# dremovd/PPO

Measured on AMD Instinct MI355X. Metric: env-steps/sec (Pong-shaped synthetic, 256 envs/GPU), higher is better.
Workload: dtype f32

## Files before the change

### ppo_amd/csrc/stack_fused.hip

```cpp
#include <cstdlib>
#include <type_traits>

#include "common.h"
#include "conv_stage.h"
#include "mfma.h"

#ifndef PPO_TAIL_SPLIT
#define PPO_TAIL_SPLIT 2
#endif

namespace ppo {
namespace {

constexpr int kScrPitchS = 20;

struct StackTailArgs {
    const float *in;
    const float *w[4];
    const float *bias[4];
    const float *mask[4];
    float *save[4];
    int n_images;
};

template <int C, int H, int W, int MT, int NW, int NSPLIT>
struct StackCfg {
    static constexpr int ROWS = H + 2;
    static constexpr int G = 4;
    static constexpr int PLANE_RAW = ROWS * W + 2 * G;
    static constexpr int PLANE = PLANE_RAW + ((16 - PLANE_RAW % 32) + 32) % 32;
    static constexpr int NT = C / 16;
    static constexpr int NTL = NT / NSPLIT;
    static constexpr int WAVES = NW * NSPLIT;
    static constexpr int KS = 9 * (C / 4);
    static constexpr int NPIX = H * W;
    static constexpr int MTILES = (NPIX + 15) / 16;
    static constexpr int LDS_MAP = C * PLANE;
    static constexpr size_t LDS_BYTES = (size_t)2 * LDS_MAP * 4;
    static_assert(C % 16 == 0, "channel tiles of 16");
    static_assert(MTILES == MT * NW, "one group of MT pixel tiles per wave");
    static_assert(NT % NSPLIT == 0, "channel tiles split evenly");
};

template <int C, int H, int W, int MT, int NW, int NSPLIT, bool BACKWARD>
__global__ __launch_bounds__(NW * NSPLIT * 64) void stack_tail_kernel(StackTailArgs a)
{
    using S = StackCfg<C, H, W, MT, NW, NSPLIT>;
    constexpr int NT = S::NTL, KS = S::KS, PLANE = S::PLANE, G = S::G;
    extern __shared__ __align__(16) float smem[];
    const int tid = threadIdx.x, lane = tid & 63, l15 = lane & 15, g = lane >> 4;
    const int wave = (tid >> 6) % NW;
    const int n0 = ((tid >> 6) / NW) * NT;

    zero_lds<2 * S::LDS_MAP, S::WAVES * 64>(smem, tid);
    __syncthreads();

    int pix[MT], lofs[MT];
    float hi_l[MT], hi_r[MT];
#pragma unroll
    for (int m = 0; m < MT; ++m) {
        const int p = (wave * MT + m) * 16 + l15;
        pix[m] = p;
        const int pc = p < S::NPIX ? p : 0;
        lofs[m] = G + pc - 1 + g * PLANE;
        hi_l[m] = (pc % W == 0) ? 0.f : INFINITY;
        hi_r[m] = (pc % W == W - 1) ? 0.f : INFINITY;
    }

    float wa[NT][KS];
    auto load_weights = [&](int layer) {
        const float4 *pw = reinterpret_cast<const float4 *>(a.w[layer]);
#pragma unroll
        for (int s4 = 0; s4 < KS / 4; ++s4)
#pragma unroll
            for (int n = 0; n < NT; ++n) {
                const float4 v = pw[(s4 * S::NT + n0 + n) * 64 + lane];
                wa[n][4 * s4 + 0] = v.x;
                wa[n][4 * s4 + 1] = v.y;
                wa[n][4 * s4 + 2] = v.z;
                wa[n][4 * s4 + 3] = v.w;
            }
    };
    load_weights(0);

    for (int img = blockIdx.x; img < a.n_images; img += gridDim.x) {
        __syncthreads();
        stage_band_chunk_dma<C, H, W, S::ROWS, PLANE, G, S::WAVES>(a.in, img, 0, smem, tid);
        const size_t img_off = (size_t)img * C * H * W;

#pragma unroll 1
        for (int layer = 0; layer < 4; ++layer) {
            float bias_r[NT][4];
#pragma unroll
            for (int n = 0; n < NT; ++n)
#pragma unroll
                for (int r = 0; r < 4; ++r) bias_r[n][r] = BACKWARD ? 0.f : a.bias[layer][(n0 + n) * 16 + g * 4 + r];
            float gate[BACKWARD ? MT : 1][NT][4];
            if constexpr (BACKWARD) {
                const __amdgpu_buffer_rsrc_t mask = buffer_of(a.mask[layer] + img_off);
#pragma unroll
                for (int m = 0; m < MT; ++m)
#pragma unroll
                    for (int n = 0; n < NT; ++n)
#pragma unroll
                        for (int r = 0; r < 4; ++r)
                            gate[m][n][r] = buffer_f32(mask, pix[m] < S::NPIX ? (((n0 + n) * 16 + g * 4 + r) * (H * W) + pix[m]) * 4
                                                                              : kOutside);
            }

            __syncthreads();
            const int odd = layer & 1;
            const int src = odd ? S::LDS_MAP : 0;
            int base[MT];
#pragma unroll
            for (int m = 0; m < MT; ++m) base[m] = lofs[m] + src;

            f32x4 acc[NT][MT];
#pragma unroll
            for (int n = 0; n < NT; ++n)
#pragma unroll
                for (int m = 0; m < MT; ++m) acc[n][m] = f32x4{0.f, 0.f, 0.f, 0.f};

            constexpr int SB = (MT * NT >= 4) ? 2 : 4;
            constexpr int NB = (KS + SB - 1) / SB;
            float raw[2][SB][MT];
            auto load_block = [&](int j, float (&r)[SB][MT]) {
#pragma unroll
                for (int u = 0; u < SB; ++u) {
                    const int s = j * SB + u;
                    if (s < KS) {
                        const int tap = s / (C / 4), cs = s % (C / 4);
                        const int tap_off = (tap / 3) * W + (tap % 3);
#pragma unroll
                        for (int m = 0; m < MT; ++m) r[u][m] = smem[base[m] + cs * 4 * PLANE + tap_off];
                    }
                }
            };
            load_block(0, raw[0]);
#pragma unroll
            for (int j = 0; j < NB; ++j) {
                float bv[SB][MT];
#pragma unroll
                for (int u = 0; u < SB; ++u) {
                    const int s = j * SB + u;
                    if (s < KS) {
                        const int kx = (s / (C / 4)) % 3;
#pragma unroll
                        for (int m = 0; m < MT; ++m) {
                            float x = raw[j & 1][u][m];
                            if (kx != 1) {
                                const float hi = kx == 0 ? hi_l[m] : hi_r[m];
                                x = __builtin_amdgcn_fmed3f(x, BACKWARD ? -hi : 0.f, hi);
                            } else if (!BACKWARD) {
                                x = relu1(x);
                            }
                            bv[u][m] = x;
                        }
                    }
                }
                __builtin_amdgcn_sched_barrier(0);
                if (j + 1 < NB) load_block(j + 1, raw[(j + 1) & 1]);
#pragma unroll
                for (int u = 0; u < SB; ++u) {
                    const int s = j * SB + u;
                    if (s < KS) {
#pragma unroll
                        for (int m = 0; m < MT; ++m)
#pragma unroll
                            for (int n = 0; n < NT; ++n) acc[n][m] = mfma16(wa[n][s], bv[u][m], acc[n][m]);
                    }
                }
                __builtin_amdgcn_sched_barrier(0);
            }

            __builtin_amdgcn_sched_barrier(0);
            load_weights((layer + 1) & 3);
            float *dst = smem + (odd ? 0 : S::LDS_MAP);
            float *save = a.save[layer];
            __builtin_amdgcn_sched_barrier(0);
            float skip[MT][NT][4];
#pragma unroll
            for (int m = 0; m < MT; ++m)
#pragma unroll
                for (int n = 0; n < NT; ++n)
#pragma unroll
                    for (int r = 0; r < 4; ++r)
                        skip[m][n][r] = odd ? smem[((n0 + n) * 16 + g * 4 + r) * PLANE + G + W + (pix[m] < S::NPIX ? pix[m] : 0)] : 0.f;
#pragma unroll
            for (int m = 0; m < MT; ++m) {
                if (pix[m] < S::NPIX) {
#pragma unroll
                    for (int n = 0; n < NT; ++n)
#pragma unroll
                        for (int r = 0; r < 4; ++r) {
                            const int co = (n0 + n) * 16 + g * 4 + r;
                            const int lo = co * PLANE + G + W + pix[m];
                            float val = acc[n][m][r] + bias_r[n][r];
                            if constexpr (BACKWARD) val = gate[m][n][r] > 0.f ? val : 0.f;
                            if (odd) val = val + skip[m][n][r];
                            dst[lo] = val;
                            if (save) save[img_off + (size_t)co * (H * W) + pix[m]] = val;
                        }
                }
            }
        }
    }
}

template <int C, int H, int W, int MT, int NW, int NSPLIT, bool BACKWARD>
int launch_stack_tail(const StackTailArgs &args, hipStream_t st)
{
    using S = StackCfg<C, H, W, MT, NW, NSPLIT>;
    constexpr auto kern = stack_tail_kernel<C, H, W, MT, NW, NSPLIT, BACKWARD>;
    int nb = 0;
    if (int rc = prepare_kernel<kern>("stack_tail", S::LDS_BYTES, S::WAVES * 64, &nb)) return rc;
    const int wg_per_cu = nb < 1 ? 1 : nb;
    int grid = 256 * wg_per_cu;
    if (grid > args.n_images) grid = args.n_images;
    hipLaunchKernelGGL(kern, dim3(grid), dim3(S::WAVES * 64), S::LDS_BYTES, st, args);
    return check_launch("stack_tail_kernel");
}

template <int C, int H, int W, int TR>
struct ShiftCfg {
    static_assert(C == 16, "one channel tile per wave");
    static constexpr int NW = 16;
    static constexpr int GW = 8;
    static constexpr int G = 4;
    static constexpr int ROWS = H + 6;
    static constexpr int PLANE_RAW = ROWS * W + 2 * G;
    static constexpr int PLANE = PLANE_RAW + ((16 - PLANE_RAW % 32) + 32) % 32;
    static constexpr int KS = 9 * (C / 4);
    static constexpr int NBANDS = (H + TR - 1) / TR;
    static constexpr int NPIX = TR * W;
    static constexpr int MTILES = (NPIX + 15) / 16;
    static constexpr int MT = MTILES / GW;
    static constexpr int LDS_MAP = C * PLANE;
    static constexpr int SCR = MT * 16 * kScrPitchS;
    static constexpr size_t LDS_BYTES = (size_t)(LDS_MAP + GW * SCR) * 4;
    static_assert(H % TR == 0 && MTILES == MT * GW, "whole bands, tiles split evenly over a group's waves");
    static_assert((H * W) % 4 == 0 && NPIX % 4 == 0 && W % 2 == 0, "float4 epilogue on whole quads");
    static_assert(LDS_BYTES <= 160 * 1024, "map + scratch must fit the CU's LDS");
};

template <int C, int H, int W, int TR, bool BACKWARD>
__global__ __launch_bounds__(1024) void stack_shift_kernel(StackTailArgs a)
{
    using S = ShiftCfg<C, H, W, TR>;
    constexpr int KS = S::KS, PLANE = S::PLANE, G = S::G, MT = S::MT, NW = S::NW;
    extern __shared__ __align__(16) float smem[];
    const int tid = threadIdx.x, lane = tid & 63, l15 = lane & 15, g = lane >> 4, wave = tid >> 6;
    const int grp = __builtin_amdgcn_readfirstlane(wave / S::GW), wv = wave % S::GW;
    const int ch = lane >> 2, quad = lane & 3;
    float *scr = smem + S::LDS_MAP + wv * S::SCR;

    int lofs[MT], p4[MT];
    float hi_l[MT], hi_r[MT];
#pragma unroll
    for (int m = 0; m < MT; ++m) {
        const int p = (wv * MT + m) * 16 + l15;
        lofs[m] = G + p - 1 + g * PLANE;
        hi_l[m] = (p % W == 0) ? 0.f : INFINITY;
        hi_r[m] = (p % W == W - 1) ? 0.f : INFINITY;
        p4[m] = (wv * MT + m) * 16 + quad * 4;
    }

    for (int img = blockIdx.x; img < a.n_images; img += gridDim.x) {
        const size_t img_off = (size_t)img * C * H * W;
        __syncthreads();
        for (int i = tid; i < C * 6 * W; i += NW * 64) {
            const int c = i / (6 * W), r = (i / W) % 6, x = i % W;
            smem[c * PLANE + G + (r < 5 ? r : H + 5) * W + x] = 0.f;
        }
        for (int i = tid; i < C * 2 * G; i += NW * 64)
            smem[(i / (2 * G)) * PLANE + ((i % (2 * G)) < G ? (i % G) : G + S::ROWS * W + (i % G))] = 0.f;
        {
            using gptr_t = const __attribute__((address_space(1))) void *;
            using lptr_t = __attribute__((address_space(3))) void *;
            constexpr int N4 = H * W / 4, REQ = (N4 + 63) / 64;
            const int w0 = __builtin_amdgcn_readfirstlane(wave);
            for (int c = w0; c < C; c += NW) {
                const float *g0 = a.in + img_off + (size_t)c * H * W;
                float *l0 = smem + c * PLANE + G + 5 * W;
#pragma unroll
                for (int q = 0; q < REQ; ++q)
                    if (q * 64 + lane < N4)
                        __builtin_amdgcn_global_load_lds((gptr_t)(g0 + (q * 64 + lane) * 4), (lptr_t)(l0 + q * 256), 16, 0, 0);
            }
        }

#pragma unroll 1
        for (int layer = 0; layer < 4; ++layer) {
            float wa[KS];
            const float4 *pw = reinterpret_cast<const float4 *>(a.w[layer]);
#pragma unroll
            for (int s4 = 0; s4 < KS / 4; ++s4) {
                const float4 v = pw[s4 * 64 + lane];
                wa[4 * s4 + 0] = v.x, wa[4 * s4 + 1] = v.y, wa[4 * s4 + 2] = v.z, wa[4 * s4 + 3] = v.w;
            }
            const float bias_c = BACKWARD ? 0.f : a.bias[layer][ch];
            const int odd = layer & 1;
            const float *res = odd ? (layer == 1 ? a.in : a.save[1]) + img_off : nullptr;
            const float *mask = BACKWARD ? a.mask[layer] + img_off : nullptr;
            float *save = a.save[layer] ? a.save[layer] + img_off : nullptr;
            const __amdgpu_buffer_rsrc_t mask_b = buffer_of(mask, mask != nullptr), res_b = buffer_of(res, res != nullptr);
            const int in_row = 5 - layer;

            f32x4 acc[MT];
            float4 gate4[MT], res4[MT];

            __syncthreads();
#pragma unroll 1
            for (int hs = 0; hs <= S::NBANDS; ++hs) {
                if ((hs & 1) == grp) {
                    if (hs < S::NBANDS) {
                        const int y0 = hs * TR;
                        const int chan_off = ch * (H * W) + y0 * W;
#pragma unroll
                        for (int m = 0; m < MT; ++m) {
                            const bool live = p4[m] < S::NPIX;
                            const int off = live ? (chan_off + p4[m]) * 4 : kOutside;
                            if constexpr (BACKWARD) gate4[m] = buffer_f32x4(mask_b, off);
                            res4[m] = buffer_f32x4(res_b, off);
                        }
                        int base[MT];
#pragma unroll
                        for (int m = 0; m < MT; ++m) {
                            base[m] = lofs[m] + (y0 - 1 + in_row) * W;
                            acc[m] = f32x4{0.f, 0.f, 0.f, 0.f};
                        }
                        constexpr int SB = 2;
                        constexpr int NB = (KS + SB - 1) / SB;
                        float raw[2][SB][MT];
                        auto load_block = [&](int j, float (&r)[SB][MT]) {
#pragma unroll
                            for (int u = 0; u < SB; ++u) {
                                const int s = j * SB + u;
                                if (s < KS) {
                                    const int tap = s / (C / 4), cs = s % (C / 4);
                                    const int tap_off = (tap / 3) * W + (tap % 3);
#pragma unroll
                                    for (int m = 0; m < MT; ++m) r[u][m] = smem[base[m] + cs * 4 * PLANE + tap_off];
                                }
                            }
                        };
                        load_block(0, raw[0]);
#pragma unroll
                        for (int j = 0; j < NB; ++j) {
                            float bv[SB][MT];
#pragma unroll
                            for (int u = 0; u < SB; ++u) {
                                const int s = j * SB + u;
                                if (s < KS) {
                                    const int kx = (s / (C / 4)) % 3;
#pragma unroll
                                    for (int m = 0; m < MT; ++m) {
                                        float x = raw[j & 1][u][m];
                                        if (kx != 1) {
                                            const float hi = kx == 0 ? hi_l[m] : hi_r[m];
                                            x = __builtin_amdgcn_fmed3f(x, BACKWARD ? -hi : 0.f, hi);
                                        } else if (!BACKWARD) {
                                            x = relu1(x);
                                        }
                                        bv[u][m] = x;
                                    }
                                }
                            }
                            __builtin_amdgcn_sched_barrier(0);
                            if (j + 1 < NB) load_block(j + 1, raw[(j + 1) & 1]);
#pragma unroll
                            for (int u = 0; u < SB; ++u) {
                                const int s = j * SB + u;
                                if (s < KS) {
#pragma unroll
                                    for (int m = 0; m < MT; ++m) acc[m] = mfma16(wa[s], bv[u][m], acc[m]);
                                }
                            }
                            __builtin_amdgcn_sched_barrier(0);
                        }
                    } else if (layer < 3) {
                        for (int i = tid % (S::GW * 64); i < C * W; i += S::GW * 64)
                            smem[(i / W) * PLANE + G + (H + in_row - 1) * W + i % W] = 0.f;
                    }
                } else if (hs >= 1) {
                    const int y0 = (hs - 1) * TR;
                    const int chan_off = ch * (H * W) + y0 * W;
#pragma unroll
                    for (int m = 0; m < MT; ++m)
#pragma unroll
                        for (int r = 0; r < 4; ++r) scr[(m * 16 + g * 4 + r) * kScrPitchS + l15] = acc[m][r];
                    __builtin_amdgcn_wave_barrier();
                    float *out_row = smem + ch * PLANE + G + (y0 + in_row - 1) * W;
#pragma unroll
                    for (int m = 0; m < MT; ++m) {
                        if (p4[m] >= S::NPIX) continue;
                        const float4 o = *reinterpret_cast<const float4 *>(scr + (m * 16 + ch) * kScrPitchS + quad * 4);
                        const float ov[4] = {o.x, o.y, o.z, o.w};
                        const float gv[4] = {gate4[m].x, gate4[m].y, gate4[m].z, gate4[m].w};
                        const float rv[4] = {res4[m].x, res4[m].y, res4[m].z, res4[m].w};
                        float v[4];
#pragma unroll
                        for (int e = 0; e < 4; ++e) {
                            float val = ov[e] + bias_c;
                            if constexpr (BACKWARD) val = gv[e] > 0.f ? val : 0.f;
                            v[e] = val + rv[e];
                        }
                        if (layer < 3) {
                            *reinterpret_cast<float2 *>(out_row + p4[m]) = make_float2(v[0], v[1]);
                            *reinterpret_cast<float2 *>(out_row + p4[m] + 2) = make_float2(v[2], v[3]);
                        }
                        if (save) *reinterpret_cast<float4 *>(save + chan_off + p4[m]) = make_float4(v[0], v[1], v[2], v[3]);
                    }
                    __builtin_amdgcn_wave_barrier();
                }
                __syncthreads();
            }
        }
    }
}

template <int C, int H, int W, int TR, bool BACKWARD>
int launch_stack_shift(const StackTailArgs &args, hipStream_t st)
{
    using S = ShiftCfg<C, H, W, TR>;
    constexpr auto kern = stack_shift_kernel<C, H, W, TR, BACKWARD>;
    if (int rc = prepare_kernel<kern>("stack_shift", S::LDS_BYTES)) return rc;
    int grid = 256;
    if (grid > args.n_images) grid = args.n_images;
    hipLaunchKernelGGL(kern, dim3(grid), dim3(S::NW * 64), S::LDS_BYTES, st, args);
    return check_launch("stack_shift_kernel");
}

template <int I, int N, class F>
__device__ __forceinline__ void static_for(F &&f)
{
    if constexpr (I < N) {
        f(std::integral_constant<int, I>{});
        static_for<I + 1, N>(f);
    }
}

struct LaneMap {
    template <int MT>
    struct T {
        int pix[MT], lofs[MT];
        float hi_l[MT], hi_r[MT];
    };
};

template <int H, int W, int PLANE, int G, int MT>
__device__ __forceinline__ void lane_map_init(LaneMap::T<MT> &lm, int pixel_wave, int l15, int g)
{
#pragma unroll
    for (int m = 0; m < MT; ++m) {
        const int p = (pixel_wave * MT + m) * 16 + l15;
        lm.pix[m] = p;
        const int pc = p < H * W ? p : 0;
        lm.lofs[m] = G + pc - 1 + g * PLANE;
        lm.hi_l[m] = (pc % W == 0) ? 0.f : INFINITY;
        lm.hi_r[m] = (pc % W == W - 1) ? 0.f : INFINITY;
    }
}

template <int C, int H, int W, int MT, int NTOT, int NT, bool RELU_IN, bool GATED = false>
__device__ __forceinline__ void resident_conv(float *smem, int src_off, int dst_off, bool residual, const float *wpk,
                                              const float *bias, float *save, const LaneMap::T<MT> &lm, int n0, int lane,
                                              const float *mask = nullptr)
{
    constexpr int ROWS = H + 2, G = 4, PLANE_RAW = ROWS * W + 2 * G;
    constexpr int PLANE = PLANE_RAW + ((16 - PLANE_RAW % 32) + 32) % 32;
    constexpr int KS = 9 * (C / 4);
    const int g = lane >> 4;
    float wa[NT][KS];
    const float4 *pw = reinterpret_cast<const float4 *>(wpk);
#pragma unroll
    for (int s4 = 0; s4 < KS / 4; ++s4)
#pragma unroll
        for (int n = 0; n < NT; ++n) {
            const float4 v = pw[(s4 * NTOT + n0 + n) * 64 + lane];
            wa[n][4 * s4 + 0] = v.x;
            wa[n][4 * s4 + 1] = v.y;
            wa[n][4 * s4 + 2] = v.z;
            wa[n][4 * s4 + 3] = v.w;
        }
    float bias_r[NT][4];
#pragma unroll
    for (int n = 0; n < NT; ++n)
#pragma unroll
        for (int r = 0; r < 4; ++r) bias_r[n][r] = (GATED || !bias) ? 0.f : bias[(n0 + n) * 16 + g * 4 + r];
    constexpr int SB = (MT * NT >= 4) ? 2 : 4;
    constexpr int NB = (KS + SB - 1) / SB;
    constexpr int GATE_AT = (GATED && MT * NT * 4 > 16) ? NB / 2 : -1;
    float gate[GATED ? MT : 1][NT][4];
    auto load_gate = [&]() {
        const __amdgpu_buffer_rsrc_t mask_b = buffer_of(mask);
#pragma unroll
        for (int m = 0; m < MT; ++m)
#pragma unroll
            for (int n = 0; n < NT; ++n)
#pragma unroll
                for (int r = 0; r < 4; ++r)
                    gate[m][n][r] = buffer_f32(mask_b, lm.pix[m] < H * W ? (((n0 + n) * 16 + g * 4 + r) * (H * W) + lm.pix[m]) * 4
                                                                         : kOutside);
    };
    if constexpr (GATED && GATE_AT < 0) load_gate();

    __syncthreads();
    int base[MT];
#pragma unroll
    for (int m = 0; m < MT; ++m) base[m] = lm.lofs[m] + src_off;
    f32x4 acc[NT][MT];
#pragma unroll
    for (int n = 0; n < NT; ++n)
#pragma unroll
        for (int m = 0; m < MT; ++m) acc[n][m] = f32x4{0.f, 0.f, 0.f, 0.f};

    float raw[2][SB][MT];
    auto load_block = [&](int j, float (&r)[SB][MT]) {
#pragma unroll
        for (int u = 0; u < SB; ++u) {
            const int s = j * SB + u;
            if (s < KS) {
                const int tap = s / (C / 4), cs = s % (C / 4);
                const int tap_off = (tap / 3) * W + (tap % 3);
#pragma unroll
                for (int m = 0; m < MT; ++m) r[u][m] = smem[base[m] + cs * 4 * PLANE + tap_off];
            }
        }
    };
    load_block(0, raw[0]);
    static_for<0, NB>([&](auto jc) {
        constexpr int j = decltype(jc)::value;
        float bv[SB][MT];
#pragma unroll
        for (int u = 0; u < SB; ++u) {
            const int s = j * SB + u;
            if (s < KS) {
                const int kx = (s / (C / 4)) % 3;
#pragma unroll
                for (int m = 0; m < MT; ++m) {
                    float x = raw[j & 1][u][m];
                    if (kx != 1) {
                        const float hi = kx == 0 ? lm.hi_l[m] : lm.hi_r[m];
                        x = __builtin_amdgcn_fmed3f(x, RELU_IN ? 0.f : -hi, hi);
                    } else if (RELU_IN) {
                        x = relu1(x);
                    }
                    bv[u][m] = x;
                }
            }
        }
        __builtin_amdgcn_sched_barrier(0);
        if constexpr (j + 1 < NB) load_block(j + 1, raw[(j + 1) & 1]);
        if constexpr (j == GATE_AT) load_gate();
#pragma unroll
        for (int u = 0; u < SB; ++u) {
            const int s = j * SB + u;
            if (s < KS) {
#pragma unroll
                for (int m = 0; m < MT; ++m)
#pragma unroll
                    for (int n = 0; n < NT; ++n) acc[n][m] = mfma16(wa[n][s], bv[u][m], acc[n][m]);
            }
        }
        __builtin_amdgcn_sched_barrier(0);
    });
#pragma unroll
    for (int m = 0; m < MT; ++m) {
        if (lm.pix[m] < H * W) {
#pragma unroll
            for (int n = 0; n < NT; ++n)
#pragma unroll
                for (int r = 0; r < 4; ++r) {
                    const int co = (n0 + n) * 16 + g * 4 + r;
                    const int lo = dst_off + co * PLANE + G + W + lm.pix[m];
                    float val = acc[n][m][r] + bias_r[n][r];
                    if constexpr (GATED) val = gate[m][n][r] > 0.f ? val : 0.f;
                    if (residual) val = val + smem[lo];
                    smem[lo] = val;
                    if (save) save[(size_t)co * (H * W) + lm.pix[m]] = val;
                }
        }
    }
}

struct StackFullArgs {
    const float *in;
    const float *w[5];
    const float *bias[5];
    float *pooled;
    uint8_t *argmax;
    float *save[4];
    const float *pre_w[4];
    const float *pre_bias[4];
    float *pre_save[4];
    int has_pre;
    int n_images;
};

template <int C, int HI, int WI, int MTI, int HO, int WO, int MTO, int NW, int NSPLIT>
__global__ __launch_bounds__(NW * NSPLIT * 64) void stack_full_kernel(StackFullArgs a)
{
    using SI = StackCfg<C, HI, WI, MTI, NW, NSPLIT>;
    using SO = StackCfg<C, HO, WO, MTO, NW, NSPLIT>;
    static_assert(HO == (HI + 1) / 2 && WO == (WI + 1) / 2, "3x3 / stride 2 / pad 1 pooling");
    static_assert(2 * SO::LDS_MAP <= SI::LDS_MAP, "the small maps reuse the input map's LDS");
    constexpr int NT = SI::NTL, WAVES = SI::WAVES, THREADS = WAVES * 64;
    constexpr int A_OFF = 0, B_OFF = SI::LDS_MAP, X_OFF = 0, Y_OFF = SO::LDS_MAP;
    extern __shared__ __align__(16) float smem[];
    const int tid = threadIdx.x, lane = tid & 63, l15 = lane & 15, g = lane >> 4;
    const int wave = tid >> 6, pixel_wave = wave % NW, n0 = (wave / NW) * NT;

    LaneMap::T<MTI> lmi;
    LaneMap::T<MTO> lmo;
    lane_map_init<HI, WI, SI::PLANE, SI::G, MTI>(lmi, pixel_wave, l15, g);
    lane_map_init<HO, WO, SO::PLANE, SO::G, MTO>(lmo, pixel_wave, l15, g);

    if (a.has_pre) zero_lds<SI::LDS_MAP, THREADS>(smem + B_OFF, tid);

    for (int img = blockIdx.x; img < a.n_images; img += gridDim.x) {
        __syncthreads();
        zero_lds<SI::LDS_MAP, THREADS>(smem + A_OFF, tid);
        __syncthreads();
        stage_band_chunk_dma<C, HI, WI, SI::ROWS, SI::PLANE, SI::G, WAVES>(a.in, img, 0, smem + A_OFF, tid);
        if (a.has_pre) {
            const size_t big_img = (size_t)img * C * HI * WI;
#pragma unroll 1
            for (int layer = 0; layer < 4; ++layer) {
                const int odd = layer & 1;
                float *save = a.pre_save[layer] ? a.pre_save[layer] + big_img : nullptr;
                resident_conv<C, HI, WI, MTI, SI::NT, NT, true>(smem, odd ? B_OFF : A_OFF, odd ? A_OFF : B_OFF, odd != 0,
                                                                a.pre_w[layer], a.pre_bias[layer], save, lmi, n0, lane);
            }
        }
        resident_conv<C, HI, WI, MTI, SI::NT, NT, false>(smem, A_OFF, B_OFF, false, a.w[0], a.bias[0], nullptr, lmi, n0, lane);
        __syncthreads();
        zero_lds<2 * SO::LDS_MAP, THREADS>(smem + X_OFF, tid);
        __syncthreads();
        {
            constexpr int RPW = 64 / WO;
            const int sub = lane / WO, xo = lane % WO;
            const size_t out_img = (size_t)img * C * HO * WO;
            for (int u0 = wave * RPW; u0 < C * HO; u0 += WAVES * RPW) {
                const int u = u0 + sub;
                const int co = u / HO, yo = u % HO;
                if (sub < RPW && co < C) {
                    const float *src = smem + B_OFF + co * SI::PLANE + SI::G + WI + (2 * yo - 1) * WI + 2 * xo - 1;
                    float best;
                    int best_tap;
                    pool_window_lds<HI % 2 == 0, WI % 2 == 0>(src, WI, yo > 0, 2 * yo + 1 < HI, xo > 0, 2 * xo + 1 < WI, best, best_tap);
                    smem[X_OFF + co * SO::PLANE + SO::G + WO + yo * WO + xo] = best;
                    const size_t oi = out_img + ((size_t)co * HO + yo) * WO + xo;
                    if (a.pooled) a.pooled[oi] = best;
                    if (a.argmax) a.argmax[oi] = (uint8_t)best_tap;
                }
            }
        }
        const size_t out_img = (size_t)img * C * HO * WO;
#pragma unroll 1
        for (int layer = 0; layer < 4; ++layer) {
            const int odd = layer & 1;
            float *save = a.save[layer] ? a.save[layer] + out_img : nullptr;
            resident_conv<C, HO, WO, MTO, SO::NT, NT, true>(smem, odd ? Y_OFF : X_OFF, odd ? X_OFF : Y_OFF, odd != 0,
                                                            a.w[1 + layer], a.bias[1 + layer], save, lmo, n0, lane);
        }
    }
}

struct StackFullBwdArgs {
    const float *g;
    const float *w[5];
    const float *mask[4];
    const uint8_t *argmax;
    float *save[4];
    float *dc;
    float *g_prev;
    const float *post_w[4];
    const float *post_mask[4];
    float *post_save[4];
    int has_post;
    int n_images;
};

template <int C, int HI, int WI, int MTI, int HO, int WO, int MTO, int NW, int NSPLIT>
__global__ __launch_bounds__(NW * NSPLIT * 64) void stack_full_bwd_kernel(StackFullBwdArgs a)
{
    using SI = StackCfg<C, HI, WI, MTI, NW, NSPLIT>;
    using SO = StackCfg<C, HO, WO, MTO, NW, NSPLIT>;
    static_assert(2 * SO::LDS_MAP <= SI::LDS_MAP, "the small maps live inside the first big map's LDS");
    static_assert(C * HO * WO <= SO::LDS_MAP * 4, "the argmax bytes of an image fit the second small map");
    constexpr int NT = SI::NTL, WAVES = SI::WAVES, THREADS = WAVES * 64;
    constexpr int A_OFF = 0, B_OFF = SI::LDS_MAP, X_OFF = 0, Y_OFF = SO::LDS_MAP;
    extern __shared__ __align__(16) float smem[];
    const int tid = threadIdx.x, lane = tid & 63, l15 = lane & 15, g = lane >> 4;
    const int wave = tid >> 6, pixel_wave = wave % NW, n0 = (wave / NW) * NT;

    LaneMap::T<MTI> lmi;
    LaneMap::T<MTO> lmo;
    lane_map_init<HI, WI, SI::PLANE, SI::G, MTI>(lmi, pixel_wave, l15, g);
    lane_map_init<HO, WO, SO::PLANE, SO::G, MTO>(lmo, pixel_wave, l15, g);

    zero_lds<SI::LDS_MAP, THREADS>(smem + B_OFF, tid);

    for (int img = blockIdx.x; img < a.n_images; img += gridDim.x) {
        __syncthreads();
        zero_lds<2 * SO::LDS_MAP, THREADS>(smem + X_OFF, tid);
        __syncthreads();
        stage_band_chunk_dma<C, HO, WO, SO::ROWS, SO::PLANE, SO::G, WAVES>(a.g, img, 0, smem + X_OFF, tid);
        const size_t small_img = (size_t)img * C * HO * WO, big_img = (size_t)img * C * HI * WI;
        constexpr int AM_WORDS = C * HO * WO / 4, AM_PER = (AM_WORDS + THREADS - 1) / THREADS;
        static_assert(C * HO * WO % 4 == 0, "an image's argmax bytes are whole words (the entry points check the base)");
        uint32_t am_r[AM_PER];
#pragma unroll
        for (int k = 0; k < AM_PER; ++k) {
            const int i = tid + k * THREADS;
            am_r[k] = reinterpret_cast<const uint32_t *>(a.argmax + small_img)[i < AM_WORDS ? i : 0];
        }
#pragma unroll 1
        for (int layer = 0; layer < 4; ++layer) {
            const int odd = layer & 1;
            resident_conv<C, HO, WO, MTO, SO::NT, NT, false, true>(smem, odd ? Y_OFF : X_OFF, odd ? X_OFF : Y_OFF, odd != 0,
                                                                   a.w[layer], nullptr, a.save[layer] + small_img, lmo, n0,
                                                                   lane, a.mask[layer] + small_img);
        }
        __syncthreads();
        const uint8_t *am = reinterpret_cast<const uint8_t *>(smem + Y_OFF);
#pragma unroll
        for (int k = 0; k < AM_PER; ++k) {
            const int i = tid + k * THREADS;
            if (i < AM_WORDS) reinterpret_cast<uint32_t *>(smem + Y_OFF)[i] = am_r[k];
        }
        __syncthreads();
        {
            for (int e = tid; e < C * HI * WI; e += THREADS) {
                const int co = e / (HI * WI), r = e % (HI * WI);
                const int iy = r / WI, ix = r % WI;
                const int k = ix >> 1, oy0 = iy >> 1;
                const int ky0 = (iy & 1) ? 2 : 1;
                const bool has_oy1 = (iy & 1) && (oy0 + 1 < HO);
                const bool odd_x = ix & 1;
                const bool has_ox1 = odd_x && (k + 1 < WO);
                const int kx0 = odd_x ? 2 : 1;
                const float *gx = smem + X_OFF + co * SO::PLANE + SO::G + WO;
                const uint8_t *ac = am + co * (HO * WO);
                float sum = 0.f;
                {
                    const int i00 = oy0 * WO + k;
                    if (ac[i00] == ky0 * 3 + kx0) sum += gx[i00];
                    if (has_ox1 && ac[i00 + 1] == ky0 * 3 + 0) sum += gx[i00 + 1];
                }
                if (has_oy1) {
                    const int i10 = (oy0 + 1) * WO + k;
                    if (ac[i10] == kx0) sum += gx[i10];
                    if (has_ox1 && ac[i10 + 1] == 0) sum += gx[i10 + 1];
                }
                smem[B_OFF + co * SI::PLANE + SI::G + WI + r] = sum;
                a.dc[big_img + e] = sum;
            }
        }
        if (a.has_post) {
            __syncthreads();
            zero_lds<SI::LDS_MAP, THREADS>(smem + A_OFF, tid);
        }
        resident_conv<C, HI, WI, MTI, SI::NT, NT, false, false>(smem, B_OFF, A_OFF, false, a.w[4], nullptr,
                                                                a.g_prev + big_img, lmi, n0, lane);
        if (a.has_post) {
#pragma unroll 1
            for (int layer = 0; layer < 4; ++layer) {
                const int odd = layer & 1;
                resident_conv<C, HI, WI, MTI, SI::NT, NT, false, true>(smem, odd ? B_OFF : A_OFF, odd ? A_OFF : B_OFF, odd != 0,
                                                                       a.post_w[layer], nullptr, a.post_save[layer] + big_img,
                                                                       lmi, n0, lane, a.post_mask[layer] + big_img);
            }
        }
    }
}

template <int C, int HI, int WI, int MTI, int HO, int WO, int MTO, int NW, int NSPLIT>
int launch_stack_full_bwd(const StackFullBwdArgs &args, hipStream_t st)
{
    using SI = StackCfg<C, HI, WI, MTI, NW, NSPLIT>;
    constexpr size_t kLds = 2 * (size_t)SI::LDS_MAP * 4;
    constexpr auto kern = stack_full_bwd_kernel<C, HI, WI, MTI, HO, WO, MTO, NW, NSPLIT>;
    if (int rc = prepare_kernel<kern>("stack_full_bwd", kLds)) return rc;
    const int grid = args.n_images < 256 ? args.n_images : 256;
    hipLaunchKernelGGL(kern, dim3(grid), dim3(SI::WAVES * 64), kLds, st, args);
    return check_launch("stack_full_bwd_kernel");
}

template <int C, int HI, int WI, int MTI, int HO, int WO, int MTO, int NW, int NSPLIT>
int launch_stack_full(const StackFullArgs &args, hipStream_t st)
{
    using SI = StackCfg<C, HI, WI, MTI, NW, NSPLIT>;
    constexpr size_t kLds = 2 * (size_t)SI::LDS_MAP * 4;
    constexpr auto kern = stack_full_kernel<C, HI, WI, MTI, HO, WO, MTO, NW, NSPLIT>;
    if (int rc = prepare_kernel<kern>("stack_full", kLds)) return rc;
    const int grid = args.n_images < 256 ? args.n_images : 256;
    hipLaunchKernelGGL(kern, dim3(grid), dim3(SI::WAVES * 64), kLds, st, args);
    return check_launch("stack_full_kernel");
}


struct ChainSplitArgs {
    const float *in;
    const float *pre_w[4];
    const float *pre_bias[4];
    const float *w[5];
    const float *bias[5];
    float *out;
    float *xbuf;
    uint32_t *flags;
    uint32_t *ctl;
    int n_images;
    int skip;
};

constexpr int kSplitWaves = 8;
constexpr uint32_t kSpinLimit = 1u << 21;

template <int C, int HI, int WI, int HO, int WO>
__global__ __launch_bounds__(kSplitWaves * 64) void stack_chain_split_kernel(ChainSplitArgs a)
{
    static_assert(C == 32, "two channel tiles: one per workgroup of a pair");
    using SI = StackCfg<C, HI, WI, 7, 4, 2>;
    using SO = StackCfg<C, HO, WO, 2, 4, 2>;
    constexpr int MTI = 4, MTO = 2, WAVES = kSplitWaves, THREADS = WAVES * 64;
    static_assert(SI::MTILES <= MTI * WAVES && SO::MTILES == MTO * 4 && WAVES == 8, "every pixel tile has a wave");
    static_assert(2 * SO::LDS_MAP <= SI::LDS_MAP, "the small maps reuse the input map's LDS");
    constexpr int A_OFF = 0, B_OFF = SI::LDS_MAP, X_OFF = 0, Y_OFF = SO::LDS_MAP;
    extern __shared__ __align__(16) float smem[];
    const int tid = threadIdx.x, lane = tid & 63, l15 = lane & 15, g = lane >> 4;
    const int wave = tid >> 6;
    const int b = blockIdx.x;
    const int h = (b >> 3) & 1;
    const int pair0 = (b & 7) | ((b >> 4) << 3);
    const int n_pairs = (gridDim.x >> 4) << 3;

    LaneMap::T<MTI> lmi;
    LaneMap::T<MTO> lmo;
    lane_map_init<HI, WI, SI::PLANE, SI::G, MTI>(lmi, wave, l15, g);
    lane_map_init<HO, WO, SO::PLANE, SO::G, MTO>(lmo, wave & 3, l15, g);

    const uint32_t base = __hip_atomic_load(a.ctl, __ATOMIC_RELAXED, __HIP_MEMORY_SCOPE_AGENT) * 8u;
    const uint32_t fault = __hip_atomic_load(a.ctl + 3, __ATOMIC_RELAXED, __HIP_MEMORY_SCOPE_AGENT);
    const uint32_t spin_limit = fault ? 1u << 10 : kSpinLimit;
    bool gave_up = false;
    zero_lds<SI::LDS_MAP, THREADS>(smem + B_OFF, tid);

    for (int img = pair0; img < a.n_images; img += n_pairs) {
        uint32_t *flag_own = a.flags + 2 * img + h, *flag_other = a.flags + 2 * img + (1 - h);
        float *slots = a.xbuf + (size_t)img * 2 * C * HI * WI;
        uint32_t step = 0;
        auto exchange = [&](int dst_off, float *slot, bool fetch) {
            ++step;
            asm volatile("s_waitcnt vmcnt(0)" ::: "memory");
            __syncthreads();
            if (tid == 0) {
                if (!(fault && h == 1))
                    __hip_atomic_store(flag_own, base + step, __ATOMIC_RELAXED, __HIP_MEMORY_SCOPE_AGENT);
                uint32_t it = 0;
                while (!(a.skip & 1) && !gave_up &&
                       __hip_atomic_load(flag_other, __ATOMIC_RELAXED, __HIP_MEMORY_SCOPE_AGENT) < base + step) {
                    if (++it > spin_limit ||
                        ((it & 1023u) == 0 && __hip_atomic_load(a.ctl + 2, __ATOMIC_RELAXED, __HIP_MEMORY_SCOPE_AGENT))) {
                        __hip_atomic_store(a.ctl + 2, 1u, __ATOMIC_RELAXED, __HIP_MEMORY_SCOPE_AGENT);
                        gave_up = true;
                        break;
                    }
                    __builtin_amdgcn_s_sleep(2);
                }
            }
            __syncthreads();
            if (fetch)
                stage_band_chunk_dma<16, HI, WI, SI::ROWS, SI::PLANE, SI::G, WAVES, 16>(slot + (size_t)(1 - h) * 16 * HI * WI, 0, 0,
                                                                                       smem + dst_off + (1 - h) * 16 * SI::PLANE, tid);
        };

        __syncthreads();
        zero_lds<SI::LDS_MAP, THREADS>(smem + A_OFF, tid);
        __syncthreads();
        stage_band_chunk_dma<C, HI, WI, SI::ROWS, SI::PLANE, SI::G, WAVES>(a.in, img, 0, smem + A_OFF, tid);
#pragma unroll 1
        for (int layer = 0; layer < 4; ++layer) {
            const int odd = layer & 1;
            float *slot = slots + (size_t)(layer & 1) * C * HI * WI;
            resident_conv<C, HI, WI, MTI, 2, 1, true>(smem, odd ? B_OFF : A_OFF, odd ? A_OFF : B_OFF, odd != 0, a.pre_w[layer],
                                                      a.pre_bias[layer], slot, lmi, h, lane);
            exchange(odd ? A_OFF : B_OFF, slot, true);
        }
        resident_conv<C, HI, WI, MTI, 2, 1, false>(smem, A_OFF, B_OFF, false, a.w[0], a.bias[0], slots, lmi, h, lane);
        exchange(B_OFF, slots, h == 0);
        if (h != 0 || (a.skip & 2)) continue;
        __syncthreads();
        zero_lds<2 * SO::LDS_MAP, THREADS>(smem + X_OFF, tid);
        __syncthreads();
        {
            constexpr int RPW = 64 / WO;
            const int sub = lane / WO, xo = lane % WO;
            for (int u0 = wave * RPW; u0 < C * HO; u0 += WAVES * RPW) {
                const int u = u0 + sub;
                const int co = u / HO, yo = u % HO;
                if (sub < RPW && co < C) {
                    const float *src = smem + B_OFF + co * SI::PLANE + SI::G + WI + (2 * yo - 1) * WI + 2 * xo - 1;
                    float best;
                    int best_tap;
                    pool_window_lds<HI % 2 == 0, WI % 2 == 0>(src, WI, yo > 0, 2 * yo + 1 < HI, xo > 0, 2 * xo + 1 < WI, best, best_tap);
                    smem[X_OFF + co * SO::PLANE + SO::G + WO + yo * WO + xo] = best;
                }
            }
        }
        float *out_img = a.out + (size_t)img * C * HO * WO;
#pragma unroll 1
        for (int layer = 0; layer < 4; ++layer) {
            const int odd = layer & 1;
            resident_conv<C, HO, WO, MTO, 2, 1, true>(smem, odd ? Y_OFF : X_OFF, odd ? X_OFF : Y_OFF, odd != 0, a.w[1 + layer],
                                                      a.bias[1 + layer], layer == 3 ? out_img : nullptr, lmo, wave >> 2, lane);
        }
    }
    __syncthreads();
    if (tid == 0) {
        const uint32_t done = __hip_atomic_fetch_add(a.ctl + 1, 1u, __ATOMIC_RELAXED, __HIP_MEMORY_SCOPE_AGENT);
        if (done == gridDim.x - 1) {
            __hip_atomic_store(a.ctl + 1, 0u, __ATOMIC_RELAXED, __HIP_MEMORY_SCOPE_AGENT);
            __hip_atomic_fetch_add(a.ctl, 1u, __ATOMIC_RELAXED, __HIP_MEMORY_SCOPE_AGENT);
        }
    }
}

template <int C, int HI, int WI, int HO, int WO>
int launch_chain_split(const ChainSplitArgs &args, hipStream_t st)
{
    using SI = StackCfg<C, HI, WI, 7, 4, 2>;
    constexpr size_t kLds = 2 * (size_t)SI::LDS_MAP * 4;
    constexpr auto kern = stack_chain_split_kernel<C, HI, WI, HO, WO>;
    if (int rc = prepare_kernel<kern>("stack_chain_split", kLds)) return rc;
// ... 329 lines not shown
```

Baseline: 98210.

## Pad LDS feature-map rows with zero columns to drop per-tap edge masking

Feature maps in LDS for the shift kernel and the full backward kernel now use a row pitch wider than the image. The pad columns hold zeros, so the 3x3 conv taps read zeros at the left and right edges and no longer need the per-element fmed3 clamping or ReLU in the MFMA inner loop. In the shift kernel, ReLU is applied once when a map is written to LDS (input staging and the epilogue) rather than on every operand read. LDS loads become volatile, with a split base register so their offsets fit the instruction's immediate field. The costs are extra LDS footprint per map, replacing the DMA global-to-LDS staging with register-staged loads, and an added full LDS zeroing at kernel start.

Result: faster. 100,900 (median of 6 runs) (+2.7%).

```diff
diff --git a/ppo_amd/csrc/stack_fused.hip b/ppo_amd/csrc/stack_fused.hip
--- a/ppo_amd/csrc/stack_fused.hip
+++ b/ppo_amd/csrc/stack_fused.hip
@@ -23,11 +23,12 @@
     int n_images;
 };
 
-template <int C, int H, int W, int MT, int NW, int NSPLIT>
+template <int C, int H, int W, int MT, int NW, int NSPLIT, int PITCH_ = W>
 struct StackCfg {
     static constexpr int ROWS = H + 2;
     static constexpr int G = 4;
-    static constexpr int PLANE_RAW = ROWS * W + 2 * G;
+    static constexpr int PITCH = PITCH_;
+    static constexpr int PLANE_RAW = ROWS * PITCH + 2 * G;
     static constexpr int PLANE = PLANE_RAW + ((16 - PLANE_RAW % 32) + 32) % 32;
     static constexpr int NT = C / 16;
     static constexpr int NTL = NT / NSPLIT;
@@ -227,8 +228,9 @@
     static constexpr int NW = 16;
     static constexpr int GW = 8;
     static constexpr int G = 4;
+    static constexpr int PITCH = W + 2;
     static constexpr int ROWS = H + 6;
-    static constexpr int PLANE_RAW = ROWS * W + 2 * G;
+    static constexpr int PLANE_RAW = ROWS * PITCH + 2 * G;
     static constexpr int PLANE = PLANE_RAW + ((16 - PLANE_RAW % 32) + 32) % 32;
     static constexpr int KS = 9 * (C / 4);
     static constexpr int NBANDS = (H + TR - 1) / TR;
@@ -247,22 +249,23 @@
 __global__ __launch_bounds__(1024) void stack_shift_kernel(StackTailArgs a)
 {
     using S = ShiftCfg<C, H, W, TR>;
-    constexpr int KS = S::KS, PLANE = S::PLANE, G = S::G, MT = S::MT, NW = S::NW;
+    constexpr int KS = S::KS, PLANE = S::PLANE, PITCH = S::PITCH, G = S::G, MT = S::MT, NW = S::NW;
     extern __shared__ __align__(16) float smem[];
     const int tid = threadIdx.x, lane = tid & 63, l15 = lane & 15, g = lane >> 4, wave = tid >> 6;
     const int grp = __builtin_amdgcn_readfirstlane(wave / S::GW), wv = wave % S::GW;
     const int ch = lane >> 2, quad = lane & 3;
     float *scr = smem + S::LDS_MAP + wv * S::SCR;
 
-    int lofs[MT], p4[MT];
-    float hi_l[MT], hi_r[MT];
+    zero_lds<S::LDS_MAP, NW * 64>(smem, tid);
+
+    int lofs[MT], p4[MT], po[MT][2];
 #pragma unroll
     for (int m = 0; m < MT; ++m) {
         const int p = (wv * MT + m) * 16 + l15;
-        lofs[m] = G + p - 1 + g * PLANE;
-        hi_l[m] = (p % W == 0) ? 0.f : INFINITY;
-        hi_r[m] = (p % W == W - 1) ? 0.f : INFINITY;
+        lofs[m] = G + (p / W) * PITCH + p % W - 1 + g * PLANE;
         p4[m] = (wv * MT + m) * 16 + quad * 4;
+        po[m][0] = (p4[m] / W) * PITCH + p4[m] % W;
+        po[m][1] = ((p4[m] + 2) / W) * PITCH + (p4[m] + 2) % W;
     }
 
     for (int img = blockIdx.x; img < a.n_images; img += gridDim.x) {
@@ -270,22 +273,25 @@
         __syncthreads();
         for (int i = tid; i < C * 6 * W; i += NW * 64) {
             const int c = i / (6 * W), r = (i / W) % 6, x = i % W;
-            smem[c * PLANE + G + (r < 5 ? r : H + 5) * W + x] = 0.f;
-        }
-        for (int i = tid; i < C * 2 * G; i += NW * 64)
-            smem[(i / (2 * G)) * PLANE + ((i % (2 * G)) < G ? (i % G) : G + S::ROWS * W + (i % G))] = 0.f;
+            smem[c * PLANE + G + (r < 5 ? r : H + 5) * PITCH + x] = 0.f;
+        }
         {
-            using gptr_t = const __attribute__((address_space(1))) void *;
-            using lptr_t = __attribute__((address_space(3))) void *;
-            constexpr int N4 = H * W / 4, REQ = (N4 + 63) / 64;
+            constexpr int W2 = W / 2, RP = 64 / W2, NQ = H / RP;
+            static_assert(H % RP == 0, "whole requests");
             const int w0 = __builtin_amdgcn_readfirstlane(wave);
+            const bool live = lane < RP * W2;
+            const int ls = live ? lane : RP * W2 - 1;
             for (int c = w0; c < C; c += NW) {
-                const float *g0 = a.in + img_off + (size_t)c * H * W;
-                float *l0 = smem + c * PLANE + G + 5 * W;
-#pragma unroll
-                for (int q = 0; q < REQ; ++q)
-                    if (q * 64 + lane < N4)
-                        __builtin_amdgcn_global_load_lds((gptr_t)(g0 + (q * 64 + lane) * 4), (lptr_t)(l0 + q * 256), 16, 0, 0);
+                const float2 *g2 = reinterpret_cast<const float2 *>(a.in + img_off + (size_t)c * H * W) + ls;
+                float *l0 = smem + c * PLANE + G + (5 + ls / W2) * PITCH + (ls % W2) * 2;
+                float2 v[NQ];
+#pragma unroll
+                for (int q = 0; q < NQ; ++q) v[q] = g2[q * RP * W2];
+#pragma unroll
+                for (int q = 0; q < NQ; ++q) {
+                    const float2 o = BACKWARD ? v[q] : make_float2(relu1(v[q].x), relu1(v[q].y));
+                    if (live) *reinterpret_cast<float2 *>(l0 + q * RP * PITCH) = o;
+                }
             }
         }
 
@@ -323,10 +329,17 @@
                             if constexpr (BACKWARD) gate4[m] = buffer_f32x4(mask_b, off);
                             res4[m] = buffer_f32x4(res_b, off);
                         }
-                        int base[MT];
+                        constexpr int CS_HI = ((C / 4 - 1) * 4 * PLANE + 2 * PITCH + 2) * 4 > 65535 ? C / 8 : C / 4;
+                        static_assert(((C / 4 - 1 - (CS_HI < C / 4 ? CS_HI : 0)) * 4 * PLANE + 2 * PITCH + 2) * 4 <= 65535 &&
+                                      ((CS_HI - 1) * 4 * PLANE + 2 * PITCH + 2) * 4 <= 65535, "operand offsets fit the instruction");
+                        using lds_cvf = const volatile __attribute__((address_space(3))) float;
+                        lds_cvf *vsmem = (lds_cvf *)smem;
+                        int base[MT], base_hi[MT];
 #pragma unroll
                         for (int m = 0; m < MT; ++m) {
-                            base[m] = lofs[m] + (y0 - 1 + in_row) * W;
+                            base[m] = lofs[m] + (y0 - 1 + in_row) * PITCH;
+                            base_hi[m] = base[m] + CS_HI * 4 * PLANE;
+                            if constexpr (CS_HI < C / 4) asm volatile("" : "+v"(base_hi[m]));
                             acc[m] = f32x4{0.f, 0.f, 0.f, 0.f};
                         }
                         constexpr int SB = 2;
@@ -338,49 +351,33 @@
                                 const int s = j * SB + u;
                                 if (s < KS) {
                                     const int tap = s / (C / 4), cs = s % (C / 4);
-                                    const int tap_off = (tap / 3) * W + (tap % 3);
-#pragma unroll
-                                    for (int m = 0; m < MT; ++m) r[u][m] = smem[base[m] + cs * 4 * PLANE + tap_off];
+                                    const int tap_off = (tap / 3) * PITCH + (tap % 3);
+#pragma unroll
+                                    for (int m = 0; m < MT; ++m)
+                                        r[u][m] = cs < CS_HI ? vsmem[base[m] + cs * 4 * PLANE + tap_off]
+                                                             : vsmem[base_hi[m] + (cs - CS_HI) * 4 * PLANE + tap_off];
                                 }
                             }
                         };
                         load_block(0, raw[0]);
 #pragma unroll
                         for (int j = 0; j < NB; ++j) {
-                            float bv[SB][MT];
+                            __builtin_amdgcn_sched_barrier(0);
+                            if (j + 1 < NB) load_block(j + 1, raw[(j + 1) & 1]);
+                            __builtin_amdgcn_sched_barrier(0);
 #pragma unroll
                             for (int u = 0; u < SB; ++u) {
                                 const int s = j * SB + u;
                                 if (s < KS) {
-                                    const int kx = (s / (C / 4)) % 3;
-#pragma unroll
-                                    for (int m = 0; m < MT; ++m) {
-                                        float x = raw[j & 1][u][m];
-                                        if (kx != 1) {
-                                            const float hi = kx == 0 ? hi_l[m] : hi_r[m];
-                                            x = __builtin_amdgcn_fmed3f(x, BACKWARD ? -hi : 0.f, hi);
-                                        } else if (!BACKWARD) {
-                                            x = relu1(x);
-                                        }
-                                        bv[u][m] = x;
-                                    }
-                                }
-                            }
-                            __builtin_amdgcn_sched_barrier(0);
-                            if (j + 1 < NB) load_block(j + 1, raw[(j + 1) & 1]);
-#pragma unroll
-                            for (int u = 0; u < SB; ++u) {
-                                const int s = j * SB + u;
-                                if (s < KS) {
-#pragma unroll
-                                    for (int m = 0; m < MT; ++m) acc[m] = mfma16(wa[s], bv[u][m], acc[m]);
+#pragma unroll
+                                    for (int m = 0; m < MT; ++m) acc[m] = mfma16(wa[s], raw[j & 1][u][m], acc[m]);
                                 }
                             }
                             __builtin_amdgcn_sched_barrier(0);
                         }
                     } else if (layer < 3) {
                         for (int i = tid % (S::GW * 64); i < C * W; i += S::GW * 64)
-                            smem[(i / W) * PLANE + G + (H + in_row - 1) * W + i % W] = 0.f;
+                            smem[(i / W) * PLANE + G + (H + in_row - 1) * PITCH + i % W] = 0.f;
                     }
                 } else if (hs >= 1) {
                     const int y0 = (hs - 1) * TR;
@@ -390,7 +387,7 @@
 #pragma unroll
                         for (int r = 0; r < 4; ++r) scr[(m * 16 + g * 4 + r) * kScrPitchS + l15] = acc[m][r];
                     __builtin_amdgcn_wave_barrier();
-                    float *out_row = smem + ch * PLANE + G + (y0 + in_row - 1) * W;
+                    float *out_row = smem + ch * PLANE + G + (y0 + in_row - 1) * PITCH;
 #pragma unroll
                     for (int m = 0; m < MT; ++m) {
                         if (p4[m] >= S::NPIX) continue;
@@ -406,8 +403,11 @@
                             v[e] = val + rv[e];
                         }
                         if (layer < 3) {
-                            *reinterpret_cast<float2 *>(out_row + p4[m]) = make_float2(v[0], v[1]);
-                            *reinterpret_cast<float2 *>(out_row + p4[m] + 2) = make_float2(v[2], v[3]);
+                            float t[4];
+#pragma unroll
+                            for (int e = 0; e < 4; ++e) t[e] = BACKWARD ? v[e] : relu1(v[e]);
+                            *reinterpret_cast<float2 *>(out_row + po[m][0]) = make_float2(t[0], t[1]);
+                            *reinterpret_cast<float2 *>(out_row + po[m][1]) = make_float2(t[2], t[3]);
                         }
                         if (save) *reinterpret_cast<float4 *>(save + chan_off + p4[m]) = make_float4(v[0], v[1], v[2], v[3]);
                     }
@@ -448,7 +448,7 @@
     };
 };
 
-template <int H, int W, int PLANE, int G, int MT>
+template <int H, int W, int PLANE, int G, int MT, int PITCH = W>
 __device__ __forceinline__ void lane_map_init(LaneMap::T<MT> &lm, int pixel_wave, int l15, int g)
 {
 #pragma unroll
@@ -456,20 +456,27 @@
         const int p = (pixel_wave * MT + m) * 16 + l15;
         lm.pix[m] = p;
         const int pc = p < H * W ? p : 0;
-        lm.lofs[m] = G + pc - 1 + g * PLANE;
-        lm.hi_l[m] = (pc % W == 0) ? 0.f : INFINITY;
-        lm.hi_r[m] = (pc % W == W - 1) ? 0.f : INFINITY;
-    }
-}
-
-template <int C, int H, int W, int MT, int NTOT, int NT, bool RELU_IN, bool GATED = false>
+        if constexpr (PITCH == W) {
+            lm.lofs[m] = G + pc - 1 + g * PLANE;
+            lm.hi_l[m] = (pc % W == 0) ? 0.f : INFINITY;
+            lm.hi_r[m] = (pc % W == W - 1) ? 0.f : INFINITY;
+        } else {
+            lm.lofs[m] = G + (pc / W) * PITCH + pc % W - 1 + g * PLANE;
+            lm.hi_l[m] = lm.hi_r[m] = 0.f;
+        }
+    }
+}
+
+template <int C, int H, int W, int MT, int NTOT, int NT, bool RELU_IN, bool GATED = false, int PITCH = W>
 __device__ __forceinline__ void resident_conv(float *smem, int src_off, int dst_off, bool residual, const float *wpk,
                                               const float *bias, float *save, const LaneMap::T<MT> &lm, int n0, int lane,
                                               const float *mask = nullptr)
 {
-    constexpr int ROWS = H + 2, G = 4, PLANE_RAW = ROWS * W + 2 * G;
+    constexpr int ROWS = H + 2, G = 4, PLANE_RAW = ROWS * PITCH + 2 * G;
     constexpr int PLANE = PLANE_RAW + ((16 - PLANE_RAW % 32) + 32) % 32;
     constexpr int KS = 9 * (C / 4);
+    constexpr bool PADDED = PITCH != W;
+    static_assert(!PADDED || (PITCH == W + 1 && !RELU_IN), "padded maps hold what the MFMA takes: identity input only");
     const int g = lane >> 4;
     float wa[NT][KS];
     const float4 *pw = reinterpret_cast<const float4 *>(wpk);
@@ -508,7 +515,10 @@
     __syncthreads();
     int base[MT];
 #pragma unroll
-    for (int m = 0; m < MT; ++m) base[m] = lm.lofs[m] + src_off;
+    for (int m = 0; m < MT; ++m) {
+        base[m] = lm.lofs[m] + src_off;
+        if constexpr (PADDED) asm volatile("" : "+v"(base[m]));
+    }
     f32x4 acc[NT][MT];
 #pragma unroll
     for (int n = 0; n < NT; ++n)
@@ -522,12 +532,20 @@
             const int s = j * SB + u;
             if (s < KS) {
                 const int tap = s / (C / 4), cs = s % (C / 4);
-                const int tap_off = (tap / 3) * W + (tap % 3);
-#pragma unroll
-                for (int m = 0; m < MT; ++m) r[u][m] = smem[base[m] + cs * 4 * PLANE + tap_off];
+                const int tap_off = (tap / 3) * PITCH + (tap % 3);
+#pragma unroll
+                for (int m = 0; m < MT; ++m) {
+                    if constexpr (PADDED) {
+                        using lds_cvf = const volatile __attribute__((address_space(3))) float;
+                        r[u][m] = ((lds_cvf *)smem)[base[m] + cs * 4 * PLANE + tap_off];
+                    } else {
+                        r[u][m] = smem[base[m] + cs * 4 * PLANE + tap_off];
+                    }
+                }
             }
         }
     };
+    static_assert(!PADDED || ((C / 4 - 1) * 4 * PLANE + 2 * PITCH + 2) * 4 <= 65535, "operand offsets fit the instruction");
     load_block(0, raw[0]);
     static_for<0, NB>([&](auto jc) {
         constexpr int j = decltype(jc)::value;
@@ -540,7 +558,8 @@
 #pragma unroll
                 for (int m = 0; m < MT; ++m) {
                     float x = raw[j & 1][u][m];
-                    if (kx != 1) {
+                    if constexpr (PADDED) {
+                    } else if (kx != 1) {
                         const float hi = kx == 0 ? lm.hi_l[m] : lm.hi_r[m];
                         x = __builtin_amdgcn_fmed3f(x, RELU_IN ? 0.f : -hi, hi);
                     } else if (RELU_IN) {
@@ -552,6 +571,7 @@
         }
         __builtin_amdgcn_sched_barrier(0);
         if constexpr (j + 1 < NB) load_block(j + 1, raw[(j + 1) & 1]);
+        if constexpr (PADDED) __builtin_amdgcn_sched_barrier(0);
         if constexpr (j == GATE_AT) load_gate();
 #pragma unroll
         for (int u = 0; u < SB; ++u) {
@@ -573,7 +593,8 @@
 #pragma unroll
                 for (int r = 0; r < 4; ++r) {
                     const int co = (n0 + n) * 16 + g * 4 + r;
-                    const int lo = dst_off + co * PLANE + G + W + lm.pix[m];
+                    const int lo = PADDED ? dst_off + co * PLANE + (lm.lofs[m] - g * PLANE) + PITCH + 1
+                                          : dst_off + co * PLANE + G + W + lm.pix[m];
                     float val = acc[n][m][r] + bias_r[n][r];
                     if constexpr (GATED) val = gate[m][n][r] > 0.f ? val : 0.f;
                     if (residual) val = val + smem[lo];
@@ -685,8 +706,8 @@
 template <int C, int HI, int WI, int MTI, int HO, int WO, int MTO, int NW, int NSPLIT>
 __global__ __launch_bounds__(NW * NSPLIT * 64) void stack_full_bwd_kernel(StackFullBwdArgs a)
 {
-    using SI = StackCfg<C, HI, WI, MTI, NW, NSPLIT>;
-    using SO = StackCfg<C, HO, WO, MTO, NW, NSPLIT>;
+    using SI = StackCfg<C, HI, WI, MTI, NW, NSPLIT, WI + 1>;
+    using SO = StackCfg<C, HO, WO, MTO, NW, NSPLIT, WO + 1>;
     static_assert(2 * SO::LDS_MAP <= SI::LDS_MAP, "the small maps live inside the first big map's LDS");
     static_assert(C * HO * WO <= SO::LDS_MAP * 4, "the argmax bytes of an image fit the second small map");
     constexpr int NT = SI::NTL, WAVES = SI::WAVES, THREADS = WAVES * 64;
@@ -697,8 +718,8 @@
 
     LaneMap::T<MTI> lmi;
     LaneMap::T<MTO> lmo;
-    lane_map_init<HI, WI, SI::PLANE, SI::G, MTI>(lmi, pixel_wave, l15, g);
-    lane_map_init<HO, WO, SO::PLANE, SO::G, MTO>(lmo, pixel_wave, l15, g);
+    lane_map_init<HI, WI, SI::PLANE, SI::G, MTI, SI::PITCH>(lmi, pixel_wave, l15, g);
+    lane_map_init<HO, WO, SO::PLANE, SO::G, MTO, SO::PITCH>(lmo, pixel_wave, l15, g);
 
     zero_lds<SI::LDS_MAP, THREADS>(smem + B_OFF, tid);
 
@@ -706,8 +727,16 @@
         __syncthreads();
         zero_lds<2 * SO::LDS_MAP, THREADS>(smem + X_OFF, tid);
         __syncthreads();
-        stage_band_chunk_dma<C, HO, WO, SO::ROWS, SO::PLANE, SO::G, WAVES>(a.g, img, 0, smem + X_OFF, tid);
         const size_t small_img = (size_t)img * C * HO * WO, big_img = (size_t)img * C * HI * WI;
+        for (int row = tid; row < C * HO; row += THREADS) {
+            const float *gr = a.g + small_img + row * WO;
+            float *lr = smem + X_OFF + (row / HO) * SO::PLANE + SO::G + (1 + row % HO) * SO::PITCH;
+            float gv[WO];
+#pragma unroll
+            for (int x = 0; x < WO; ++x) gv[x] = gr[x];
+#pragma unroll
+            for (int x = 0; x < WO; ++x) lr[x] = gv[x];
+        }
         constexpr int AM_WORDS = C * HO * WO / 4, AM_PER = (AM_WORDS + THREADS - 1) / THREADS;
         static_assert(C * HO * WO % 4 == 0, "an image's argmax bytes are whole words (the entry points check the base)");
         uint32_t am_r[AM_PER];
@@ -719,7 +748,7 @@
 #pragma unroll 1
         for (int layer = 0; layer < 4; ++layer) {
             const int odd = layer & 1;
-            resident_conv<C, HO, WO, MTO, SO::NT, NT, false, true>(smem, odd ? Y_OFF : X_OFF, odd ? X_OFF : Y_OFF, odd != 0,
+            resident_conv<C, HO, WO, MTO, SO::NT, NT, false, true, SO::PITCH>(smem, odd ? Y_OFF : X_OFF, odd ? X_OFF : Y_OFF, odd != 0,
                                                                    a.w[layer], nullptr, a.save[layer] + small_img, lmo, n0,
                                                                    lane, a.mask[layer] + small_img);
         }
@@ -741,20 +770,20 @@
                 const bool odd_x = ix & 1;
                 const bool has_ox1 = odd_x && (k + 1 < WO);
                 const int kx0 = odd_x ? 2 : 1;
-                const float *gx = smem + X_OFF + co * SO::PLANE + SO::G + WO;
+                const float *gx = smem + X_OFF + co * SO::PLANE + SO::G + SO::PITCH;
                 const uint8_t *ac = am + co * (HO * WO);
                 float sum = 0.f;
                 {
-                    const int i00 = oy0 * WO + k;
-                    if (ac[i00] == ky0 * 3 + kx0) sum += gx[i00];
-                    if (has_ox1 && ac[i00 + 1] == ky0 * 3 + 0) sum += gx[i00 + 1];
+                    const int i00 = oy0 * WO + k, x00 = oy0 * SO::PITCH + k;
+                    if (ac[i00] == ky0 * 3 + kx0) sum += gx[x00];
+                    if (has_ox1 && ac[i00 + 1] == ky0 * 3 + 0) sum += gx[x00 + 1];
                 }
                 if (has_oy1) {
-                    const int i10 = (oy0 + 1) * WO + k;
-                    if (ac[i10] == kx0) sum += gx[i10];
-                    if (has_ox1 && ac[i10 + 1] == 0) sum += gx[i10 + 1];
-                }
-                smem[B_OFF + co * SI::PLANE + SI::G + WI + r] = sum;
+                    const int i10 = (oy0 + 1) * WO + k, x10 = (oy0 + 1) * SO::PITCH + k;
+                    if (ac[i10] == kx0) sum += gx[x10];
+                    if (has_ox1 && ac[i10 + 1] == 0) sum += gx[x10 + 1];
+                }
+                smem[B_OFF + co * SI::PLANE + SI::G + (1 + iy) * SI::PITCH + ix] = sum;
                 a.dc[big_img + e] = sum;
             }
         }
@@ -762,13 +791,13 @@
             __syncthreads();
             zero_lds<SI::LDS_MAP, THREADS>(smem + A_OFF, tid);
         }
-        resident_conv<C, HI, WI, MTI, SI::NT, NT, false, false>(smem, B_OFF, A_OFF, false, a.w[4], nullptr,
+        resident_conv<C, HI, WI, MTI, SI::NT, NT, false, false, SI::PITCH>(smem, B_OFF, A_OFF, false, a.w[4], nullptr,
                                                                 a.g_prev + big_img, lmi, n0, lane);
         if (a.has_post) {
 #pragma unroll 1
             for (int layer = 0; layer < 4; ++layer) {
                 const int odd = layer & 1;
-                resident_conv<C, HI, WI, MTI, SI::NT, NT, false, true>(smem, odd ? B_OFF : A_OFF, odd ? A_OFF : B_OFF, odd != 0,
+                resident_conv<C, HI, WI, MTI, SI::NT, NT, false, true, SI::PITCH>(smem, odd ? B_OFF : A_OFF, odd ? A_OFF : B_OFF, odd != 0,
                                                                        a.post_w[layer], nullptr, a.post_save[layer] + big_img,
                                                                        lmi, n0, lane, a.post_mask[layer] + big_img);
             }
@@ -779,8 +808,9 @@
 template <int C, int HI, int WI, int MTI, int HO, int WO, int MTO, int NW, int NSPLIT>
 int launch_stack_full_bwd(const StackFullBwdArgs &args, hipStream_t st)
 {
-    using SI = StackCfg<C, HI, WI, MTI, NW, NSPLIT>;
+    using SI = StackCfg<C, HI, WI, MTI, NW, NSPLIT, WI + 1>;
     constexpr size_t kLds = 2 * (size_t)SI::LDS_MAP * 4;
+    static_assert(kLds <= 160 * 1024, "two padded maps fit the CU's LDS");
     constexpr auto kern = stack_full_bwd_kernel<C, HI, WI, MTI, HO, WO, MTO, NW, NSPLIT>;
     if (int rc = prepare_kernel<kern>("stack_full_bwd", kLds)) return rc;
     const int grid = args.n_images < 256 ? args.n_images : 256;
```
